# danini/multi-h

Measured on AMD Instinct MI355X. Metric: scored homography hypotheses/sec (50k pts x 100k models), higher is better.
Workload: dtype f64

## Files before the change

multi-h_amd/csrc/capi_label.hip:

```cpp
#include "capi_engine.hpp"

namespace {

int expand_contexts(const mh_engine* e)
{
    const int want = std::max(1, std::min(e->tune_expand_ctx, EXPAND_MAX_CTX));
    const double per_ctx = 4.0 * (2.0 * (double)e->g_nnz + 13.0 * (double)e->n + 2048.0);
    const int fit = 1 + (int)std::min(64.0, 8.0 * 1024.0 * 1024.0 * 1024.0 / std::max(per_ctx, 1.0));
    return std::max(1, std::min(want, fit));
}

int ensure_expand_work(mh_engine* e)
{
    const int n = e->n, n_ctx = expand_contexts(e);
    HIPCHK(e->ew_label.reserve(n));
    HIPCHK(e->ew_cur.reserve(n));
    HIPCHK(e->h_flags.ensure(EXPAND_HOST_WORDS));
    HIPCHK(e->h_acc.ensure(16));
    for (int k = 0; k < n_ctx; ++k) HIPCHK(e->ew_ctx[k].reserve(n, e->g_nnz, n_ctx > 1, e->stream));
    if (n_ctx > 1) {
        HIPCHK(e->ew_bctl.reserve(8 + EXPAND_MAX_CTX));
        HIPCHK(e->h_batch.ensure(8));
    }
    return MH_OK;
}

int do_data_cost(mh_engine* e)
{
    const int L = e->m + 1;
    HIPCHK(e->cost.reserve((size_t)e->n * L));
    {
        ScopedTimer t(e, MH_K_DATACOST);
        HIPCHK(launch_data_cost(e->pts(), e->H.p, e->m, e->lambda, e->thr_H * e->thr_H, e->cost.p, e->stream,
                                e->data_term == MH_DATA_TERM_RISING));
    }
    e->cost_L = L;
    return MH_OK;
}

int solve_grid_limit(mh_engine* e)
{
    if (e->solve_grid_max > 0) return MH_OK;
    int per_cu = 0;
    HIPCHK(solver_blocks_per_cu(&per_cu));
    if (per_cu < 1) return fail(MH_ERR_HIP, "the alpha-expansion solver kernel does not fit a compute unit");
    e->solve_grid_max = e->cu_count * 1;
    return MH_OK;
}

int do_expand(mh_engine* e, const int* init_dev, long long* energy, int* cycles)
{
    if (!e->have_graph) return fail(MH_ERR_NOT_SET, "neighbour graph is not set");
    if (e->cost_L != e->m + 1) return fail(MH_ERR_NOT_SET, "data cost is stale; call mh_data_cost first");
    int rc = ensure_expand_work(e);
    if (rc) return rc;
    Graph g{ e->d_rowptr.p, e->d_col.p, e->d_w.p, e->d_rev.p, e->n, e->g_nnz, e->d_order.p, e->d_wsum.p };
    rc = solve_grid_limit(e);
    if (rc) return rc;
    int solve_grid = std::max(1, std::min(e->tune_expand[3], e->solve_grid_max));
    ExpandWork w;
    w.label = e->ew_label.p; w.cur_cost = e->ew_cur.p;
    w.n_ctx = expand_contexts(e);
    for (int k = 0; k < w.n_ctx; ++k) w.ctx[k] = e->ew_ctx[k].view(g.n, g.nnz);
    w.h_flags = e->h_flags.h; w.h_flags_dev = e->h_flags.d;
    w.h_acc = e->h_acc.h; w.h_acc_dev = e->h_acc.d;
    if (w.n_ctx > 1) {
        w.bctl = e->ew_bctl.p;
        w.h_batch = e->h_batch.h; w.h_batch_dev = e->h_batch.d;
    }
    ExpandTuning& tu = w.tune;
    tu.relax_rounds = e->tune_expand[0]; tu.push_cycles = e->tune_expand[1]; tu.push_phases = e->tune_expand[2];
    tu.push_mult = e->tune_push_mult;
    tu.reduce_rounds = e->tune_reduce; tu.reduce_launches = e->tune_reduce_launches;
    tu.cascade_iters = e->tune_cascade_iters;
    tu.batch_min_labels = e->tune_batch_min_labels; tu.batch_spw = e->tune_batch_spw;
    const size_t recycle_words = (size_t)e->cost_L * ((size_t)g.nnz + (size_t)g.n);
    if (e->tune_recycle && recycle_words <= ((size_t)2 << 30)) {
        HIPCHK(e->ew_saved.reserve(recycle_words));
        HIPCHK(hipMemsetAsync(e->ew_saved.p, 0, sizeof(int) * recycle_words, e->stream));
        w.saved_flow = e->ew_saved.p;
        w.saved_sink = e->ew_saved.p + (size_t)e->cost_L * g.nnz;
    }
    if (e->trace_moves > 0) {
        HIPCHK(e->ew_trace.reserve(8 * (size_t)e->trace_moves + 4 * 2048));
        HIPCHK(hipMemsetAsync(e->ew_trace.p, 0, sizeof(int) * (8 * (size_t)e->trace_moves + 4 * 2048), e->stream));
        w.detail_move = e->detail_move;
        w.trace = e->ew_trace.p;
        w.trace_moves = e->trace_moves;
    }
    if (e->comp_moves > 0) {
        HIPCHK(e->ew_comp.reserve(2 * (size_t)g.n));
        HIPCHK(e->ew_comp_out.reserve(16 * (size_t)e->comp_moves));
        HIPCHK(hipMemsetAsync(e->ew_comp_out.p, 0, sizeof(int) * 16 * (size_t)e->comp_moves, e->stream));
        w.comp_out = e->ew_comp_out.p; w.comp_scratch = e->ew_comp.p; w.comp_moves = e->comp_moves;
    }
    const int potts = (int)std::round(100.0 * e->lambda);
    ExpandStats st{};
    {
        ScopedTimer t(e, MH_K_EXPAND);
        ExpandResult res;
        e->last_expand_retries = 0;
        for (int attempt = 0; attempt < 5; ++attempt) {
            tu.solve_grid = solve_grid;
            const bool last_attempt = attempt == 4 || solve_grid == 1;
            const double steady_ms = std::max(20.0, 50.0 * e->longest_barrier_wait_ms);
            tu.barrier_timeout_ticks = last_attempt ? 300000000ll : (long long)(steady_ms * 1e5);
            tu.barrier_first_timeout_ticks = last_attempt ? 300000000ll : (long long)(std::max(250.0, 10.0 * steady_ms) * 1e5);
            if (w.saved_flow) HIPCHK(hipMemsetAsync(e->ew_saved.p, 0, sizeof(int) * recycle_words, e->stream));
            HIPCHK(launch_init_labeling(e->cost.p, e->cost_L, e->n, init_dev, w.label, w.cur_cost, e->stream));
            w.hooks.inject_group = e->inject_solve_failure >> 4;
            w.hooks.inject_ctx = e->inject_solve_failure & 15;
            e->inject_solve_failure = 0;
            res = run_expansion(g, e->cost.p, e->cost_L, potts, w, 1000, &st, e->stream);
            if (res.status == ExpandStatus::ok && e->inject_barrier_timeouts > 0) {
                --e->inject_barrier_timeouts;
                res.status = ExpandStatus::barrier_timeout;
            }
            e->last_solve_grid = solve_grid;
            if (res.status != ExpandStatus::barrier_timeout || solve_grid == 1 || attempt == 4) break;
            if (attempt >= 1) solve_grid = std::max(1, solve_grid / 2);
            ++e->last_expand_retries;
            ++e->expand_retries_total;
        }
        switch (res.status) {
        case ExpandStatus::ok: break;
        case ExpandStatus::too_many_sites:
            return fail(MH_ERR_INVALID, "alpha-expansion: more sites than the solver's per-row state holds (about 1.3 million at 256 workgroups)");
        case ExpandStatus::overflow:
            return fail(MH_ERR_OVERFLOW, "int32 energy term overflow in alpha-expansion");
        case ExpandStatus::barrier_timeout:
            return fail(MH_ERR_HIP, "alpha-expansion: the solver's grid barrier timed out even with the launch cut down to a few workgroups "
                                    "(its workgroups were not all resident; is the GPU shared with other persistent launches?)");
        case ExpandStatus::no_convergence:
            return fail(MH_ERR_HIP, "alpha-expansion: push-relabel did not converge within its iteration bound");
        case ExpandStatus::hip_error: { const hipError_t he = res.hip; HIPCHK(he); }
        }
    }
    e->last_expand = st;
    if (st.max_barrier_wait_ms > e->longest_barrier_wait_ms) e->longest_barrier_wait_ms = std::min(st.max_barrier_wait_ms, 50.0);
    if (st.energy > 0x7fffffffll || st.energy < -0x7fffffffll)
        return fail(MH_ERR_OVERFLOW, "total energy exceeds the reference's int32 EnergyType");
    if (energy) *energy = st.energy;
    if (cycles) *cycles = st.cycles;
    return MH_OK;
}

__global__ void k_shift_labels(int n, const int* in, int delta, int* out)
{
    const int i = blockIdx.x * 256 + threadIdx.x;
    if (i < n) out[i] = in[i] + delta;
}

}

extern "C" {

static int compat_trial_stats(mh_engine* e, const double* pts_xyxy, const int* cluster_begin, int clusters, const int* tri,
                              const double* H, const unsigned char* ok, const double* F, int trials, double* stats_out, double* H_out,
                              unsigned char* ok_out)
{
    if (!e) return fail(MH_ERR_INVALID, "null engine");
    if (clusters < 0 || trials < 0) return fail(MH_ERR_INVALID, "negative cluster or trial count");
    if (clusters == 0 || trials == 0) return MH_OK;
    if (!pts_xyxy || !cluster_begin || !tri || !stats_out || (!F && (!H || !ok))) return fail(MH_ERR_INVALID, "null argument");
    if (cluster_begin[0] != 0) return fail(MH_ERR_INVALID, "cluster_begin[0] must be 0");
    for (int c = 0; c < clusters; ++c)
        if (cluster_begin[c + 1] - cluster_begin[c] < 19)
            return fail(MH_ERR_INVALID, "a cluster of fewer than 19 points: the caller handles those itself (the three stale entries of the reference's buffer reach the median ranks)");
    const size_t total = (size_t)cluster_begin[clusters], ct = (size_t)clusters * (size_t)trials;
    if (ct > (size_t)0x7fffffff) return fail(MH_ERR_INVALID, "too many trials");
    for (size_t i = 0; i < ct; ++i) {
        const int nc = cluster_begin[i / trials + 1] - cluster_begin[i / trials];
        for (int j = 0; j < 3; ++j)
            if (tri[3 * i + j] < 0 || tri[3 * i + j] >= nc) return fail(MH_ERR_INVALID, "a trial draws a point outside its cluster");
    }
    HIPCHK(hipSetDevice(e->device));
    HIPCHK(e->cp_pts.reserve(4 * total)); HIPCHK(e->cp_begin.reserve(clusters + 1)); HIPCHK(e->cp_tri.reserve(3 * ct));
    HIPCHK(e->cp_H.reserve(9 * ct)); HIPCHK(e->cp_ok.reserve(ct)); HIPCHK(e->cp_out.reserve(8 * ct));
    HIPCHK(hipMemcpyAsync(e->cp_pts.p, pts_xyxy, sizeof(double) * 4 * total, hipMemcpyHostToDevice, e->stream));
    HIPCHK(hipMemcpyAsync(e->cp_begin.p, cluster_begin, sizeof(int) * (clusters + 1), hipMemcpyHostToDevice, e->stream));
    HIPCHK(hipMemcpyAsync(e->cp_tri.p, tri, sizeof(int) * 3 * ct, hipMemcpyHostToDevice, e->stream));
    if (F) {
        HIPCHK(launch_compat_fit(e->cp_pts.p, e->cp_begin.p, clusters, e->cp_tri.p, F, trials, e->cp_H.p, e->cp_ok.p, e->stream));
    } else {
        HIPCHK(hipMemcpyAsync(e->cp_H.p, H, sizeof(double) * 9 * ct, hipMemcpyHostToDevice, e->stream));
        HIPCHK(hipMemcpyAsync(e->cp_ok.p, ok, ct, hipMemcpyHostToDevice, e->stream));
    }
    HIPCHK(launch_compat_select(e->cp_pts.p, e->cp_begin.p, clusters, e->cp_tri.p, e->cp_H.p, e->cp_ok.p, trials, e->cp_out.p, e->stream));
    HIPCHK(hipMemcpyAsync(stats_out, e->cp_out.p, sizeof(double) * 8 * ct, hipMemcpyDeviceToHost, e->stream));
    if (H_out) HIPCHK(hipMemcpyAsync(H_out, e->cp_H.p, sizeof(double) * 9 * ct, hipMemcpyDeviceToHost, e->stream));
    if (ok_out) HIPCHK(hipMemcpyAsync(ok_out, e->cp_ok.p, ct, hipMemcpyDeviceToHost, e->stream));
    HIPCHK(hipStreamSynchronize(e->stream));
    return MH_OK;
}

int mh_compat_trial_stats(mh_engine* e, const double* pts_xyxy, const int* cluster_begin, int clusters, const int* tri,
                          const double* H, const unsigned char* ok, int trials, double* stats_out)
{
    return guarded([&]() -> int {
    if (!H || !ok) return fail(MH_ERR_INVALID, "null argument");
    return compat_trial_stats(e, pts_xyxy, cluster_begin, clusters, tri, H, ok, nullptr, trials, stats_out, nullptr, nullptr);
    });
}

int mh_compat_trial_stats_fit(mh_engine* e, const double* pts_xyxy, const int* cluster_begin, int clusters, const int* tri,
                              const double F[9], int trials, double* stats_out, double* H_out, unsigned char* ok_out)
{
    return guarded([&]() -> int {
    if (!F) return fail(MH_ERR_INVALID, "null argument");
    return compat_trial_stats(e, pts_xyxy, cluster_begin, clusters, tri, nullptr, nullptr, F, trials, stats_out, H_out, ok_out);
    });
}

int mh_data_cost(mh_engine* e, int* cost)
{
    return guarded([&]() -> int {
    int rc = require_models(e);
    if (rc) return rc;
    rc = do_data_cost(e);
    if (rc) return rc;
    if (cost) {
        HIPCHK(hipMemcpyAsync(cost, e->cost.p, sizeof(int) * (size_t)e->n * e->cost_L, hipMemcpyDeviceToHost, e->stream));
        HIPCHK(hipStreamSynchronize(e->stream));
    }
    return MH_OK;
    });
}

int mh_expand(mh_engine* e, const int* init_labels, int* labels_out, int* energy, int* cycles)
{
    return guarded([&]() -> int {
    int rc = require_models(e);
    if (rc) return rc;
    const int* init_dev = nullptr;
    if (init_labels) {
        for (int i = 0; i < e->n; ++i)
            if (init_labels[i] < 0 || init_labels[i] > e->m)
                return fail(MH_ERR_INVALID, "initial label out of range 0..Nh");
        HIPCHK(e->labels_in.reserve(e->n));
        HIPCHK(hipMemcpyAsync(e->labels_in.p, init_labels, sizeof(int) * e->n, hipMemcpyHostToDevice, e->stream));
        init_dev = e->labels_in.p;
    }
    long long en = 0;
    rc = do_expand(e, init_dev, &en, cycles);
    if (rc) return rc;
    if (energy) *energy = (int)en;
    if (labels_out) {
        HIPCHK(hipMemcpyAsync(labels_out, e->ew_label.p, sizeof(int) * e->n, hipMemcpyDeviceToHost, e->stream));
        HIPCHK(hipStreamSynchronize(e->stream));
    }
    return MH_OK;
    });
}

int mh_get_expand_stats(mh_engine* e, long long stats[24])
{
    return guarded([&]() -> int {
    if (!e || !stats) return fail(MH_ERR_INVALID, "null argument");
    const ExpandStats& x = e->last_expand;
    stats[0] = x.cycles;
    stats[1] = x.moves;
    stats[2] = x.accepted;
    stats[3] = x.push_phases;
    stats[4] = x.relax_intervals;
    stats[5] = x.host_syncs;
    stats[6] = x.reduce_launches;
    stats[7] = x.flow_moves;
    stats[8] = x.launches;
    stats[9] = x.moves_run;
    stats[10] = x.moves_solved;
    stats[11] = x.core_sites;
    stats[12] = x.core_max;
    stats[13] = x.barriers;
    stats[14] = x.outer_iterations;
    stats[15] = (long long)(x.solve_ms * 1000.0);
    stats[16] = (long long)(x.barrier_ms * 1000.0);
    stats[17] = (long long)(x.relax_ms * 1000.0);
    stats[18] = (long long)(x.push_ms * 1000.0);
    stats[19] = (long long)(x.tail_ms * 1000.0);
    stats[20] = e->last_expand_retries;
    stats[21] = e->last_solve_grid;
    stats[22] = e->expand_retries_total;
    stats[23] = (long long)(e->last_expand.max_barrier_wait_ms * 1e3);
    return MH_OK;
    });
}

int mh_get_expand_batch_stats(mh_engine* e, long long stats[8])
{
    return guarded([&]() -> int {
    if (!e || !stats) return fail(MH_ERR_INVALID, "null argument");
    const ExpandStats& x = e->last_expand;
    stats[0] = x.batches;
    stats[1] = x.batch_committed;
    stats[2] = x.batch_invalid;
    stats[3] = x.host_skipped;
    stats[4] = x.solo_moves;
    stats[5] = x.injected_discarded;
    stats[6] = expand_contexts(e);
    stats[7] = e->tune_batch_min_labels;
    return MH_OK;
    });
}

int mh_get_expand_trace(mh_engine* e, int* trace, int moves)
{
    return guarded([&]() -> int {
    int rc = enter(e);
    if (rc) return rc;
    if (!trace || moves <= 0) return fail(MH_ERR_INVALID, "null trace or moves <= 0");
    if (e->trace_moves <= 0 || !e->ew_trace.p) return fail(MH_ERR_NOT_SET, "tracing is off (mh_set_tuning key 8) or no expansion has run");
    const int m = std::min(moves, (int)std::min<size_t>((size_t)e->trace_moves + 1024, e->ew_trace.cap / 8));
    HIPCHK(hipMemcpyAsync(trace, e->ew_trace.p, sizeof(int) * 8 * (size_t)m, hipMemcpyDeviceToHost, e->stream));
    HIPCHK(hipStreamSynchronize(e->stream));
    return MH_OK;
    });
}

int mh_get_core_components(mh_engine* e, int* out, int moves)
{
    return guarded([&]() -> int {
    int rc = enter(e);
    if (rc) return rc;
    if (!out || moves <= 0) return fail(MH_ERR_INVALID, "null output or moves <= 0");
    if (e->comp_moves <= 0 || !e->ew_comp_out.p) return fail(MH_ERR_NOT_SET, "the component diagnostic is off (mh_set_tuning key 21) or no expansion has run");
    const int m = std::min(moves, (int)(e->ew_comp_out.cap / 16));
    HIPCHK(hipMemcpyAsync(out, e->ew_comp_out.p, sizeof(int) * 16 * (size_t)m, hipMemcpyDeviceToHost, e->stream));
    HIPCHK(hipStreamSynchronize(e->stream));
    return MH_OK;
    });
}

}

namespace mhe {

int launch_estimator(mh_engine* e, const int* labels_dev, int Nh, double* H_dev, int* counts_dev)
{
    ScopedTimer t(e, MH_K_REESTIMATE);
    if (e->estimator == MH_ESTIMATOR_3PT) {
        HIPCHK(e->r3_scratch.reserve(reestimate_3pt_scratch_ints(e->n, Nh)));
        HIPCHK(launch_reestimate_3pt(e->pts(), labels_dev, Nh, e->epi, H_dev, counts_dev, e->r3_scratch.p, e->stream,
                                     e->tune_3pt_form));
        return MH_OK;
    }
    Affines a{ e->a11.p, e->a12.p, e->a21.p, e->a22.p };
    HIPCHK(launch_reestimate(e->pts(), a, labels_dev, Nh, e->epi, H_dev, counts_dev, e->stream));
    return MH_OK;
}

}

extern "C" {

int mh_set_estimator(mh_engine* e, int estimator)
{
    return guarded([&]() -> int {
    int rc = enter(e);
    if (rc) return rc;
    if (estimator != MH_ESTIMATOR_HAF && estimator != MH_ESTIMATOR_3PT) return fail(MH_ERR_INVALID, "unknown estimator");
    e->estimator = estimator;
    return MH_OK;
    });
}

int mh_set_data_term(mh_engine* e, int term)
{
    return guarded([&]() -> int {
    if (!e) return fail(MH_ERR_INVALID, "null engine");
    if (term != MH_DATA_TERM_REFERENCE && term != MH_DATA_TERM_RISING) return fail(MH_ERR_INVALID, "unknown data term");
    e->data_term = term;
    e->cost_L = 0;
    return MH_OK;
    });
}

int mh_reestimate(mh_engine* e, const int* labels, double* H_out)
{
    return guarded([&]() -> int {
    int rc = require_models(e);
    if (rc) return rc;
    if (!labels) return fail(MH_ERR_INVALID, "labels is null");
    if (e->estimator == MH_ESTIMATOR_HAF && !e->have_aff) return fail(MH_ERR_NOT_SET, "affinities are not set");
    if (!e->have_epi) return fail(MH_ERR_NOT_SET, "fundamental matrix / epipole are not set");
    HIPCHK(e->labels_pts.reserve(e->n));
    HIPCHK(e->label_counts.reserve(e->m));
    HIPCHK(hipMemcpyAsync(e->labels_pts.p, labels, sizeof(int) * e->n, hipMemcpyHostToDevice, e->stream));
    rc = launch_estimator(e, e->labels_pts.p, e->m, e->H.p, e->label_counts.p);
    if (rc) return rc;
    e->cost_L = 0;
    if (H_out) {
        HIPCHK(hipMemcpyAsync(H_out, e->H.p, sizeof(double) * 9 * e->m, hipMemcpyDeviceToHost, e->stream));
        HIPCHK(hipStreamSynchronize(e->stream));
    }
    return MH_OK;
    });
}

int mh_labeling_step(mh_engine* e, int warm, int* labeling, double* energy, int* cycles)
{
    return guarded([&]() -> int {
    int rc = require_models(e);
    if (rc) return rc;
    if (!labeling) return fail(MH_ERR_INVALID, "labeling is null");
    if (e->estimator == MH_ESTIMATOR_HAF && (!e->have_aff || !e->have_epi))
        return fail(MH_ERR_NOT_SET, "affinities / epipolar geometry are not set");
    if (!e->have_epi) return fail(MH_ERR_NOT_SET, "epipolar geometry is not set");
    rc = do_data_cost(e);
    if (rc) return rc;
    const int* init_dev = nullptr;
    const dim3 grid((e->n + 255) / 256), blk(256);
    if (warm) {
        for (int i = 0; i < e->n; ++i)
            if (labeling[i] < -1 || labeling[i] >= e->m)
                return fail(MH_ERR_INVALID, "warm-start label out of range -1..Nh-1");
        HIPCHK(e->labels_in.reserve(e->n));
        HIPCHK(hipMemcpyAsync(e->labels_in.p, labeling, sizeof(int) * e->n, hipMemcpyHostToDevice, e->stream));
        hipLaunchKernelGGL(k_shift_labels, grid, blk, 0, e->stream, e->n, e->labels_in.p, 1, e->labels_in.p);
        init_dev = e->labels_in.p;
    }
    long long en = 0;
    rc = do_expand(e, init_dev, &en, cycles);
    if (rc) return rc;
    HIPCHK(e->labels_pts.reserve(e->n));
    HIPCHK(e->label_counts.reserve(e->m));
    hipLaunchKernelGGL(k_shift_labels, grid, blk, 0, e->stream, e->n, e->ew_label.p, -1, e->labels_pts.p);
    rc = launch_estimator(e, e->labels_pts.p, e->m, e->H.p, e->label_counts.p);
    if (rc) return rc;
    e->cost_L = 0;
    HIPCHK(hipMemcpyAsync(labeling, e->labels_pts.p, sizeof(int) * e->n, hipMemcpyDeviceToHost, e->stream));
    HIPCHK(hipStreamSynchronize(e->stream));
    if (energy) *energy = (double)en;
    return MH_OK;
    });
}

}
```

multi-h_amd/csrc/expand.hip:

```cpp

#include "expand_ctl.hpp"
#include "expand_plan.hpp"

#include <algorithm>
#include <atomic>
#include <chrono>

namespace mh {

__global__ void k_ctl_init(MoveBatch b)
{
    int* flags = b.c[blockIdx.x].flags;
    long long* acc = b.c[blockIdx.x].acc;
    for (int t = threadIdx.x; t < C_COUNT; t += blockDim.x) flags[t] = (t == C_TLAST || t == C_PEND) ? -1 : 0;
    for (int t = threadIdx.x; t < A_TOTAL; t += blockDim.x) acc[t] = 0;
}

__global__ void __launch_bounds__(256)
k_init_labeling(const int* __restrict__ cost, int L, int n, const int* __restrict__ init,
                int* __restrict__ label, int* __restrict__ cur_cost)
{
    const int i = blockIdx.x * 256 + threadIdx.x;
    if (i >= n) return;
    const int l = init ? init[i] : 0;
    label[i] = l;
    cur_cost[i] = cost[(size_t)i * L + l];
}

__global__ void __launch_bounds__(256)
k_argmin_labels(const int* __restrict__ cost, int L, int n, int* __restrict__ label,
                long long* __restrict__ acc)
{
    const int i = blockIdx.x * 256 + threadIdx.x;
    long long mine = 0;
    if (i < n) {
        int best = 0, bc = cost[(size_t)i * L];
        for (int l = 1; l < L; ++l) {
            const int c = cost[(size_t)i * L + l];
            if (c < bc) { bc = c; best = l; }
        }
        label[i] = best;
        mine = bc;
    }
    __shared__ long long s[256];
    s[threadIdx.x] = mine;
    __syncthreads();
    for (int st = 128; st >= 1; st >>= 1) {
        if ((int)threadIdx.x < st) s[threadIdx.x] += s[threadIdx.x + st];
        __syncthreads();
    }
    if (threadIdx.x == 0)
        atomicAdd((unsigned long long*)&acc[A_ENERGY_S + (blockIdx.x % STRIPES) * STRIPE_LL], (unsigned long long)s[0]);
}

constexpr int LPN = 16;
constexpr int SITES_PER_BLOCK = 256 / LPN;


template <typename F>
__device__ __forceinline__ void for_flagged(unsigned long long mask, F body)
{
    const int grp = (int)(threadIdx.x & 63) / LPN;
    while (mask) {
        int b[4];
#pragma unroll
        for (int q = 0; q < 4; ++q) {
            b[q] = mask ? (int)__builtin_ctzll(mask) : -1;
            if (mask) mask &= mask - 1;
        }
        const int m = grp == 0 ? b[0] : grp == 1 ? b[1] : grp == 2 ? b[2] : b[3];
        body(m);
    }
}
constexpr int SPW = 16;
constexpr int SPW_MAX = 64;
constexpr int SITES_PER_WBLOCK_MAX = 4 * SPW_MAX;

__global__ void __launch_bounds__(256)
k_move_setup(Graph g, const int* __restrict__ cost, int L, int potts, int reduce_on,
             int* label, int* __restrict__ cur_cost, MoveBatch b, int spw)
{
    const MoveCtx& c = b.c[blockIdx.y];
    const int alpha = c.alpha, t = c.t;
    const unsigned char* __restrict__ took = c.took;
    int* __restrict__ cap = c.cap;
    int* __restrict__ excess = c.excess;
    int* __restrict__ sink_cap = c.sink_cap;
    int* __restrict__ decided = c.decided;
    int* __restrict__ flags = c.flags;
    long long* __restrict__ acc = c.acc;
    const int lane = threadIdx.x & 63;
    const int sub = threadIdx.x % LPN;
    const int s0 = (blockIdx.x * 4 + (int)(threadIdx.x >> 6)) * spw;
    const int i = s0 + lane;
    const bool in = lane < spw && i < g.n;
    const int pa = flags[C_PEND];
    int li = 0, cc = 0;
    if (in) {
        li = label[i];
        cc = cur_cost[i];
        if (pa >= 0 && took[i]) {
            li = pa;
            cc = cost[(size_t)i * L + pa];
            label[i] = pa; cur_cost[i] = cc;
        }
    }
    if (__shfl(move_is_skipped(flags, t, L) ? 1 : 0, 0)) return;
    long long K = 0;
    bool walk = false;
    if (in) {
        if (li == alpha) decided[i] = 3;
        else {
            K = cost[(size_t)i * L + alpha];
            if (reduce_on && K - cc > 2ll * potts * g.wsum[i]) decided[i] = 2;
            else walk = true;
        }
    }
    for_flagged(__ballot(walk), [&](int m) {
        const int mm = m < 0 ? 0 : m;
        const int li_m = __shfl(li, mm), cc_m = __shfl(cc, mm);
        const long long K_m = __shfl(K, mm);
        if (m < 0) return;
        const int im = s0 + m;
        const int k0 = g.rowptr[im], k1 = g.rowptr[im + 1];
        long long S = 0, out = 0, inn = 0;
        for (int k = k0 + sub; k < k1; k += LPN) {
            const int j = g.col[k];
            const long long wk64 = (long long)g.w[k] * potts;
            if (wk64 > 0x7fffffffll) atomicExch(&flags[C_ERROR], ERR_OVERFLOW);
            const int wk = wk64 > 0x7fffffffll ? 0x7fffffff : (int)wk64;
            int lj = label[j];
            if (pa >= 0 && took[j]) lj = pa;
            if (lj == alpha) { S += wk; cap[k] = 0; cap[g.rev[k]] = 0; }
            else if (j < im) { if (li_m != lj) S += wk; cap[k] = wk; out += wk; if (li_m == lj) inn += wk; }
            else { const int c = (li_m == lj) ? wk : 0; cap[k] = c; out += c; inn += wk; }
        }
        S = row_sum64<LPN>(S) + cc_m;
        out = row_sum64<LPN>(out);
        inn = row_sum64<LPN>(inn);
        if (sub != 0) return;
        const long long tr = S - K_m;
        if (tr > 0x7fffffffll || -tr > 0x7fffffffll) atomicExch(&flags[C_ERROR], ERR_OVERFLOW);
        const int ex = tr > 0 ? (int)tr : 0;
        excess[im] = ex;
        sink_cap[im] = tr < 0 ? (int)(-tr) : 0;
        int verdict = 0;
        if (reduce_on) {
            if (tr > out) verdict = 1;
            else if (-tr > inn) verdict = 2;
        }
        decided[im] = verdict;
        if (ex > 0) atomicAdd((unsigned long long*)&acc[A_EXCESS_S + (blockIdx.x % STRIPES) * STRIPE_LL], (unsigned long long)ex);
    });
}

template <bool COMPACT>
__global__ void __launch_bounds__(256)
k_reduce(Graph g, int L, MoveBatch b, int ROUNDS, int housekeep, int spw)
{
    const MoveCtx& c = b.c[blockIdx.y];
    const int t = c.t;
    int* cap = c.cap;
    int* excess = c.excess;
    int* sink_cap = c.sink_cap;
    int* decided = c.decided;
    int* __restrict__ flags = c.flags;
    long long* __restrict__ acc = c.acc;
    int* __restrict__ core = c.core;
    const int lane = threadIdx.x & 63;
    const int sub = threadIdx.x % LPN;
    const int slot = (blockIdx.x * 4 + (int)(threadIdx.x >> 6)) * spw + lane;
    const int u = (lane < spw && slot < g.n) ? (COMPACT ? g.order[slot] : slot) : -1;
    __shared__ int s_skip;
    __shared__ int s_cnt, s_base;
    __shared__ int s_list[SITES_PER_WBLOCK_MAX];
    if (threadIdx.x == 0) { s_skip = move_is_skipped(flags, t, L) ? 1 : 0; s_cnt = 0; }
    __syncthreads();
    const bool skipped = s_skip != 0;
    if (housekeep && blockIdx.x == 0 && threadIdx.x == 0) {
        flags[C_PEND] = -1;
        flags[C_TICKET] = 0;
        flags[C_TOOK_N] = 0;
        for (int s = 0; s < SUBTICKETS; ++s) flags[C_SUBTICKET + s * C_LINE] = 0;
        long long ex = 0;
        for (int s = 0; s < STRIPES; ++s) { ex += acc[A_EXCESS_S + s * STRIPE_LL]; acc[A_EXCESS_S + s * STRIPE_LL] = 0; acc[A_DELTA_S + s * STRIPE_LL] = 0; }
        if (!skipped && ex > 0x7fffffffll) flags[C_ERROR] = ERR_OVERFLOW;
    }
    if (skipped) return;
    const bool open = u >= 0 && LD(&decided[u]) == 0;
    for_flagged(__ballot(open), [&](int m) {
        const int um = __shfl(u, m < 0 ? 0 : m);
        if (m < 0) return;
        const int k0 = g.rowptr[um], k1 = g.rowptr[um + 1];
        long long net = (long long)excess[um] - sink_cap[um];
        bool dirty = false;
        int verdict = 0;
        for (int r = 0; r < ROUNDS; ++r) {
            long long add = 0, out = 0, in = 0;
            for (int k = k0 + sub; k < k1; k += LPN) {
                const int kr = g.rev[k];
                const int co = cap[k], ci = cap[kr];
                if ((co | ci) == 0) continue;
                const int dv = LD(&decided[g.col[k]]);
                if (dv == 1) { add += ci; cap[k] = 0; cap[kr] = 0; }
                else if (dv == 2) { add -= co; cap[k] = 0; cap[kr] = 0; }
                else { out += co; in += ci; }
            }
            add = row_sum64<LPN>(add); out = row_sum64<LPN>(out); in = row_sum64<LPN>(in);
            if (add != 0) { net += add; dirty = true; }
            if (net > out) verdict = 1;
            else if (-net > in) verdict = 2;
            if (verdict) break;
        }
        if (sub == 0) {
            if (dirty) {
                if (net > 0x7fffffffll || -net > 0x7fffffffll) atomicExch(&flags[C_ERROR], ERR_OVERFLOW);
                excess[um] = net > 0 ? (int)net : 0;
                sink_cap[um] = net < 0 ? (int)(-net) : 0;
            }
            if (verdict) ST(&decided[um], verdict);
            else if (COMPACT) s_list[atomicAdd(&s_cnt, 1)] = um;
        }
    });
    if (COMPACT) {
        __syncthreads();
        const int shard = blockIdx.x % EXPAND_CORE_SHARDS;
        if (threadIdx.x == 0 && s_cnt > 0) s_base = atomicAdd(&flags[C_CORE + shard], s_cnt);
        __syncthreads();
        if ((int)threadIdx.x < s_cnt) core[(size_t)shard * g.n + s_base + threadIdx.x] = s_list[threadIdx.x];
    }
}

__global__ void __launch_bounds__(1024)
k_core_components(Graph g, int L, int t, const int* __restrict__ decided, const int* __restrict__ flags, int* __restrict__ comp,
                  int* __restrict__ csize, int* __restrict__ out)
{
    __shared__ int s_changed, s_acc[16];
    if (threadIdx.x < 16) { s_acc[threadIdx.x] = 0; out[threadIdx.x] = 0; }
    if (move_is_skipped(flags, t, L)) return;
    for (int i = threadIdx.x; i < g.n; i += 1024) { comp[i] = decided[i] == 0 ? i : -1; csize[i] = 0; }
    __syncthreads();
    int rounds = 0;
    for (;;) {
        if (threadIdx.x == 0) s_changed = 0;
        __syncthreads();
        for (int i = threadIdx.x; i < g.n; i += 1024) {
            int c = comp[i];
            if (c < 0) continue;
            int m = c;
            for (int k = g.rowptr[i]; k < g.rowptr[i + 1]; ++k) { const int cj = comp[g.col[k]]; if (cj >= 0 && cj < m) m = cj; }
            if (m < c) { atomicMin(&comp[i], m); atomicMin(&comp[c], m); s_changed = 1; }
        }
        __syncthreads();
        for (int i = threadIdx.x; i < g.n; i += 1024) {
            int c = comp[i];
            if (c < 0) continue;
            while (comp[c] < c) c = comp[c];
            comp[i] = c;
        }
        __syncthreads();
        ++rounds;
        if (!s_changed || rounds > 4096) break;
        __syncthreads();
    }
    for (int i = threadIdx.x; i < g.n; i += 1024) if (comp[i] >= 0) { atomicAdd(&csize[comp[i]], 1); atomicAdd(&s_acc[0], 1); }
    __syncthreads();
    for (int i = threadIdx.x; i < g.n; i += 1024) {
        const int sz = csize[i];
        if (sz <= 0) continue;
        atomicAdd(&s_acc[1], 1);
        const int old = atomicMax(&s_acc[2], sz);
        atomicMax(&s_acc[3], old < sz ? old : sz);
        if (sz <= 64) { atomicAdd(&s_acc[4], sz); atomicAdd(&s_acc[9], 1); }
        if (sz <= 256) { atomicAdd(&s_acc[5], sz); atomicAdd(&s_acc[10], 1); }
        if (sz <= 1024) { atomicAdd(&s_acc[6], sz); atomicAdd(&s_acc[11], 1); }
        if (sz <= 2048) { atomicAdd(&s_acc[7], sz); atomicAdd(&s_acc[12], 1); }
        if (sz <= 8192) { atomicAdd(&s_acc[8], sz); atomicAdd(&s_acc[13], 1); }
    }
    __syncthreads();
    if (threadIdx.x < 16) out[threadIdx.x] = threadIdx.x == 14 ? rounds : s_acc[threadIdx.x];
}

__global__ void __launch_bounds__(256)
k_delta(Graph g, const int* __restrict__ cost, int L, int potts,
        const int* __restrict__ label, const int* __restrict__ cur_cost, MoveBatch b, int spw)
{
    const MoveCtx& c = b.c[blockIdx.y];
    const int alpha = c.alpha, t = c.t;
    const int* __restrict__ decided = c.decided;
    unsigned char* __restrict__ took = c.took;
    int* __restrict__ flags = c.flags;
    long long* acc = c.acc;
    __shared__ long long s[256];
    __shared__ int s_last;
    if (threadIdx.x == 0) s_last = move_is_skipped(flags, t, L) ? 1 : 0;
    __syncthreads();
    if (s_last) return;
    const int lane = threadIdx.x & 63;
    const int sub = threadIdx.x % LPN;
    const int s0 = (blockIdx.x * 4 + (int)(threadIdx.x >> 6)) * spw;
    const int i = s0 + lane;
    long long mine = 0;
    int oi = 0;
    bool ti = false;
    if (lane < spw && i < g.n) {
        oi = label[i];
        ti = decided[i] == 1;
        took[i] = ti ? 1 : 0;
        if (ti) mine += (long long)cost[(size_t)i * L + alpha] - cur_cost[i];
    }
    if (c.took_list) {
        const unsigned long long tb = __ballot(ti);
        if (tb) {
            int base = 0;
            if (lane == 0) base = atomicAdd(&flags[C_TOOK_N], (int)__popcll(tb));
            base = __shfl(base, 0);
            if (ti) c.took_list[base + (int)__popcll(tb & ((1ull << lane) - 1ull))] = i;
        }
    }
    for_flagged(__ballot(ti), [&](int m) {
        const int oi_m = __shfl(oi, m < 0 ? 0 : m);
        if (m < 0) return;
        const int im = s0 + m;
        for (int k = g.rowptr[im] + sub; k < g.rowptr[im + 1]; k += LPN) {
            const int j = g.col[k];
            const bool tj = decided[j] == 1;
            if (tj && j > im) continue;
            const int oj = label[j];
            const int nj = tj ? alpha : oj;
            const int dn = (alpha != nj) - (oi_m != oj);
            mine += (long long)dn * g.w[k] * potts;
        }
    });
    s[threadIdx.x] = mine;
    __syncthreads();
    for (int st = 128; st >= 1; st >>= 1) {
        if ((int)threadIdx.x < st) s[threadIdx.x] += s[threadIdx.x + st];
        __syncthreads();
    }
    if (threadIdx.x == 0) {
        if (s[0] != 0) atomicAdd((unsigned long long*)&acc[A_DELTA_S + (blockIdx.x % STRIPES) * STRIPE_LL], (unsigned long long)s[0]);
        asm volatile("s_waitcnt vmcnt(0)" ::: "memory");
        const int st = (int)(blockIdx.x % SUBTICKETS);
        const int members = ((int)gridDim.x - st + SUBTICKETS - 1) / SUBTICKETS;
        int last = 0;
        if (atomicAdd(&flags[C_SUBTICKET + st * C_LINE], 1) == members - 1) {
            const int used = (int)gridDim.x < SUBTICKETS ? (int)gridDim.x : SUBTICKETS;
            last = atomicAdd(&flags[C_TICKET], 1) == used - 1;
        }
        s_last = last;
    }
    __syncthreads();
    if (s_last && threadIdx.x < 64) {
        long long d = (int)threadIdx.x < STRIPES ? LD(&acc[A_DELTA_S + threadIdx.x * STRIPE_LL]) : 0ll;
#pragma unroll
        for (int m = 32; m >= 1; m >>= 1) d += __shfl_xor(d, m, 64);
        if (threadIdx.x == 0 && d < 0) {
            flags[C_TLAST] = t;
            flags[C_PEND] = alpha;
            flags[C_ACCEPTED] += 1;
        }
        if (threadIdx.x == 0) {
            flags[C_MOVES_RUN] += 1;
            for (int s = 0; s < EXPAND_CORE_SHARDS; ++s) flags[C_CORE + s] = 0;
            for (int s = C_XCD; s < C_TOP + C_LINE; ++s) flags[s] = 0;
            flags[C_ARRIVE] = 0;
        }
    }
}

__global__ void __launch_bounds__(256)
k_apply_pending(int n, const int* __restrict__ cost, int L, int* __restrict__ label,
                int* __restrict__ cur_cost, const unsigned char* __restrict__ took,
                const int* __restrict__ flags, int )
{
    const int pa = flags[C_PEND];
    if (pa < 0) return;
    const int i = blockIdx.x * 256 + threadIdx.x;
    if (i < n && took[i]) {
        label[i] = pa;
        cur_cost[i] = cost[(size_t)i * L + pa];
    }
}



__global__ void k_batch_prep(MoveBatch b, int* __restrict__ bctl)
{
    int* G = b.c[0].flags;
    const int k = threadIdx.x;
    if (k == 0) { bctl[B_TLAST0] = G[C_TLAST]; G[C_PEND] = -1; }
    if (k < EXPAND_MAX_CTX) bctl[B_BAD + k] = 0;
    if (k >= 1 && k < b.count) {
        int* f = b.c[k].flags;
        f[C_TLAST] = G[C_TLAST];
        f[C_PEND] = -1;
        f[C_ERROR] = G[C_ERROR];
    }
}

__device__ __forceinline__ bool batch_move_skipped(const MoveCtx& c, int tlast0, int L)
{
    return c.flags[C_ERROR] != 0 || (c.t >= L && tlast0 <= c.t - L);
}

__global__ void __launch_bounds__(256)
k_batch_check(Graph g, const int* __restrict__ cost, int L, int potts, const int* __restrict__ label, const int* __restrict__ cur_cost,
              MoveBatch b, int* __restrict__ bctl)
{
    const int j = blockIdx.y;
    if (j + 1 >= b.count) return;
    const MoveCtx& cj = b.c[j];
    const int tlast0 = bctl[B_TLAST0];
    if (batch_move_skipped(cj, tlast0, L) || cj.flags[C_PEND] < 0) return;
    const int nt = cj.flags[C_TOOK_N];
    const int sub = threadIdx.x % LPN;
    const int alpha_j = cj.alpha, later = b.count - 1 - j;
    unsigned bad = 0;
    for (int idx = blockIdx.x * SITES_PER_BLOCK + (int)threadIdx.x / LPN; idx < nt; idx += gridDim.x * SITES_PER_BLOCK) {
        const int p = cj.took_list[idx];
        const int k0 = g.rowptr[p], k1 = g.rowptr[p + 1];
        for (int a = k0 + sub - (sub == 0 ? 1 : 0); a < k1; a = (a < k0 ? k0 : a + LPN)) {
            const int s_ = a < k0 ? p : g.col[a];
            const long long W = (long long)potts * g.wsum[s_];
            const int lb = label[s_];
            const long long Dl = cur_cost[s_];
            const int* row = cost + (size_t)s_ * L + (alpha_j + 1);
            const long long Dj = a < k0 ? (long long)cost[(size_t)s_ * L + alpha_j] : 0;
            for (int q = 0; q < later; ++q) {
                const long long Db = row[q];
                bool ok = lb == alpha_j + 1 + q || Db - Dl > W;
                if (ok && a < k0) ok = Db - Dj > W;
                if (!ok) bad |= 1u << (j + 1 + q);
            }
        }
    }
#pragma unroll
    for (int m = 32; m >= 1; m >>= 1) bad |= (unsigned)__shfl_xor((int)bad, m, 64);
    if ((threadIdx.x & 63) == 0 && bad) atomicOr((unsigned*)&bctl[B_BAD + j], bad);
}

struct CtxFlags { int* p[EXPAND_MAX_CTX]; };
__global__ void __launch_bounds__(256)
k_batch_commit(const int* __restrict__ cost, int L, int* __restrict__ label, int* __restrict__ cur_cost, MoveBatch b,
               int* __restrict__ bctl, int* __restrict__ h_batch, CtxFlags all_flags, int n_ctx_all)
{
    __shared__ int s_first, s_err, s_last_t, s_n_acc;
    __shared__ unsigned s_acc;
    __shared__ int s_ek[EXPAND_MAX_CTX], s_pend[EXPAND_MAX_CTX], s_nt[EXPAND_MAX_CTX];
    __shared__ unsigned s_bad[EXPAND_MAX_CTX];
    __shared__ int s_g[5];
    if ((int)threadIdx.x < b.count) {
        const int* f = b.c[threadIdx.x].flags;
        s_ek[threadIdx.x] = f[C_ERROR];
        s_pend[threadIdx.x] = f[C_PEND];
        s_nt[threadIdx.x] = f[C_TOOK_N];
        s_bad[threadIdx.x] = (unsigned)bctl[B_BAD + threadIdx.x];
    } else if (threadIdx.x >= 64 && threadIdx.x < 69) {
        const int q = threadIdx.x - 64;
        const int* G = b.c[0].flags;
        s_g[q] = q == 0 ? bctl[B_TLAST0] : q == 1 ? G[C_ERROR] : q == 2 ? G[C_TLAST] : q == 3 ? G[C_ACCEPTED] : bctl[B_SEQ];
    }
    __syncthreads();
    if (threadIdx.x == 0) {
        const int tlast0 = s_g[0];
        unsigned accepted = 0;
        int first_invalid = b.count, err = 0, last_t = -1, n_acc = 0;
        for (int k = 0; k < b.count; ++k) {
            const MoveCtx& c = b.c[k];
            const int ek = s_ek[k];
            const bool skipped = ek != 0 || (c.t >= L && tlast0 <= c.t - L);
            bool valid = true;
            if (accepted) {
                if (skipped) valid = false;
                else
                    for (int j = 0; j < k; ++j)
                        if ((accepted >> j & 1u) && (s_bad[j] >> k & 1u)) valid = false;
            }
            if (!valid) { first_invalid = k; break; }
            if (ek) err = ek;
            if (!skipped && s_pend[k] >= 0) { accepted |= 1u << k; last_t = c.t; ++n_acc; }
        }
        s_first = first_invalid; s_err = err; s_acc = accepted; s_last_t = last_t; s_n_acc = n_acc;
    }
    __syncthreads();
    const unsigned accepted = s_acc;
    for (int k = 0; k < b.count; ++k) {
        if (!(accepted >> k & 1u)) continue;
        const MoveCtx& c = b.c[k];
        const int nt = s_nt[k], a = c.alpha;
        for (int i = blockIdx.x * 256 + threadIdx.x; i < nt; i += gridDim.x * 256) {
            const int p = c.took_list[i];
            label[p] = a;
            cur_cost[p] = cost[(size_t)p * L + a];
        }
    }
    __shared__ int s_is_last;
    __syncthreads();
    if (threadIdx.x == 0) {
        __threadfence();
        s_is_last = atomicAdd(&bctl[B_TICKET], 1) == (int)gridDim.x - 1;
    }
    __syncthreads();
    if (s_is_last && threadIdx.x == 0) {
        bctl[B_TICKET] = 0;
        int* G = b.c[0].flags;
        const int g_err = s_g[1] ? s_g[1] : s_err;
        const int g_tlast = s_last_t > s_g[2] ? s_last_t : s_g[2];
        const int seq = s_g[4] + 1;
        if (g_err != s_g[1]) G[C_ERROR] = g_err;
        if (g_tlast != s_g[2]) G[C_TLAST] = g_tlast;
        G[C_ACCEPTED] = s_g[3] + s_n_acc - (int)(accepted & 1u);
        bctl[B_SEQ] = seq;
        h_batch[HB_FIRST_INVALID] = s_first;
        h_batch[HB_TLAST] = g_tlast;
        h_batch[HB_ERROR] = g_err;
        h_batch[HB_ACCEPTED_HERE] = s_n_acc;
        h_batch[HB_DIRTY] = 0;
        __threadfence_system();
        __hip_atomic_store(&h_batch[HB_SEQ], seq, __ATOMIC_RELEASE, __HIP_MEMORY_SCOPE_SYSTEM);
        bctl[B_TLAST0] = g_tlast;
        G[C_PEND] = -1;
        for (int k = 0; k < EXPAND_MAX_CTX; ++k) bctl[B_BAD + k] = 0;
        for (int k = 1; k < n_ctx_all; ++k) {
            int* f = all_flags.p[k];
            f[C_TLAST] = g_tlast;
            f[C_PEND] = -1;
            f[C_ERROR] = g_err;
        }
    }
}

__global__ void k_stats_merge(MoveBatch b)
{
    const int t = threadIdx.x;
    int* G = b.c[0].flags;
    long long* A = b.c[0].acc;
    const int fw[5] = { C_FLOW_MOVES, C_MOVES_SOLVED, C_MOVES_RUN, C_CORE_MAX, C_XCD_USED };
    if (t < 5) {
        const int w = fw[t];
        int v = G[w];
        for (int k = 1; k < b.count; ++k) {
            int* f = b.c[k].flags;
            if (t < 3) v += f[w]; else if (f[w] > v) v = f[w];
            f[w] = 0;
        }
        G[w] = v;
    } else if (t >= 8 && t - 8 + A_CORE_SUM < A_COUNT) {
        const int w = t - 8 + A_CORE_SUM;
        long long v = A[w];
        for (int k = 1; k < b.count; ++k) {
            long long* a = b.c[k].acc;
            if (w == A_MAX_WAIT) { if (a[w] > v) v = a[w]; } else v += a[w];
            a[w] = 0;
        }
        A[w] = v;
    }
}

__global__ void __launch_bounds__(256)
k_energy(Graph g, int potts, const int* __restrict__ label, const int* __restrict__ cur_cost,
         int* __restrict__ flags, long long* __restrict__ acc)
{
    if (blockIdx.x == 0 && threadIdx.x == 0) flags[C_PEND] = -1;
    const int i = blockIdx.x * SITES_PER_BLOCK + threadIdx.x / LPN;
    const int sub = threadIdx.x % LPN;
    long long mine = 0;
    if (i < g.n) {
        if (sub == 0) mine = cur_cost[i];
        const int li = label[i];
        for (int k = g.rowptr[i] + sub; k < g.rowptr[i + 1]; k += LPN) {
            const int j = g.col[k];
            if (j < i && label[j] != li) mine += (long long)g.w[k] * potts;
        }
    }
    __shared__ long long s[256];
    s[threadIdx.x] = mine;
    __syncthreads();
    for (int st = 128; st >= 1; st >>= 1) {
        if ((int)threadIdx.x < st) s[threadIdx.x] += s[threadIdx.x + st];
        __syncthreads();
    }
    if (threadIdx.x == 0)
        atomicAdd((unsigned long long*)&acc[A_ENERGY_S + (blockIdx.x % STRIPES) * STRIPE_LL], (unsigned long long)s[0]);
}

hipError_t launch_init_labeling(const int* cost, int L, int n, const int* init, int* label,
                                int* cur_cost, hipStream_t s)
{
    hipLaunchKernelGGL(k_init_labeling, dim3((n + 255) / 256), dim3(256), 0, s, cost, L, n, init,
                       label, cur_cost);
    return hipGetLastError();
}

hipError_t launch_argmin_labels(const int* cost, int L, int n, int* label, long long* acc,
                                hipStream_t s)
{
    hipLaunchKernelGGL(k_argmin_labels, dim3((n + 255) / 256), dim3(256), 0, s, cost, L, n, label,
                       acc);
    return hipGetLastError();
}

__global__ void k_publish(const int* __restrict__ flags, long long* __restrict__ acc,
                          int* __restrict__ h_flags, long long* __restrict__ h_acc)
{
    const int t = threadIdx.x;
    if (t < EXPAND_HOST_WORDS) h_flags[t] = flags[t];
    long long en = t < STRIPES ? acc[A_ENERGY_S + t * STRIPE_LL] : 0ll;
    if (t < STRIPES) acc[A_ENERGY_S + t * STRIPE_LL] = 0;
#pragma unroll
    for (int m = 32; m >= 1; m >>= 1) en += __shfl_xor(en, m, 64);
    if (t < A_COUNT) h_acc[t] = t == A_ENERGY ? en : acc[t];
}

namespace {

ExpandResult hip_failed(hipError_t e) { return ExpandResult{ ExpandStatus::hip_error, e }; }
#define RET_IF(x) do { hipError_t e_ = (x); if (e_ != hipSuccess) return hip_failed(e_); } while (0)

struct Launcher {
    hipStream_t s;
    ExpandStats& stats;
    template <class... P, class... A>
    void operator()(void (*k)(P...), dim3 grid, dim3 blk, A&&... a) { ++stats.launches; uncounted(k, grid, blk, a...); }
    template <class... P, class... A>
    void uncounted(void (*k)(P...), dim3 grid, dim3 blk, A&&... a) { hipLaunchKernelGGL(k, grid, blk, 0, s, a...); }
    void solve(const SolveLaunch& sl, const Graph& g, int L, const MoveBatch& b, const SolveParams& sp)
    {
        ++stats.launches;
        launch_solve(sl, g, L, b, sp, s);
    }
};

hipError_t fetch(const ExpandWork& w, Launcher& launch)
{
    ++launch.stats.host_syncs;
    launch(k_publish, dim3(1), dim3(64), w.ctx[0].flags, w.ctx[0].acc, w.h_flags_dev, w.h_acc_dev);
    hipError_t e = hipGetLastError();
    return e != hipSuccess ? e : hipStreamSynchronize(launch.s);
}

hipError_t await_commit(const int* h_batch, int batch_seq, hipStream_t s)
{
    const volatile int* seq_word = h_batch + HB_SEQ;
    const auto t_poll = std::chrono::steady_clock::now();
    bool seen = false;
    for (int spin = 0;; ++spin) {
        if (*seq_word == batch_seq) { seen = true; break; }
        if ((spin & 255) == 255 && std::chrono::steady_clock::now() - t_poll > std::chrono::milliseconds(2)) break;
    }
    if (seen) std::atomic_thread_fence(std::memory_order_acquire);
    else if (hipError_t e = hipStreamSynchronize(s); e != hipSuccess) return e;
    return h_batch[HB_SEQ] == batch_seq ? hipSuccess : hipErrorUnknown;
}

ExpandStatus status_of(int err_word)
{
    return err_word == ERR_OVERFLOW ? ExpandStatus::overflow : err_word == ERR_BARRIER_TIMEOUT ? ExpandStatus::barrier_timeout
                                                                                               : ExpandStatus::no_convergence;
}

}

ExpandResult run_expansion(const Graph& g, const int* cost, int L, int potts, ExpandWork& w,
                           int max_cycles, ExpandStats* st, hipStream_t s)
{
    const ExpandTuning& tu = w.tune;
    const dim3 grid1((g.n + 255) / 256), blk(256);
    const dim3 grid((g.n + SITES_PER_BLOCK - 1) / SITES_PER_BLOCK);
    auto spw_for = [&](int count) {
        if (tu.batch_spw == 16 || tu.batch_spw == 32 || tu.batch_spw == 64) return tu.batch_spw;
        const long long site_moves = (long long)count * g.n;
        return site_moves > (1ll << 19) ? 64 : site_moves > (1ll << 18) ? 32 : 16;
    };
    ExpandStats stats = {};
    Launcher launch{ s, stats };
    auto ended = [&](ExpandStatus status) { if (st) *st = stats; return ExpandResult{ status, hipSuccess }; };
    const int n_ctx = std::max(1, std::min(w.n_ctx, EXPAND_MAX_CTX));
    MoveBatch all{};
    all.count = n_ctx;
    CtxFlags all_flags{};
    for (int k = 0; k < n_ctx; ++k) {
        const ExpandWork::Ctx& x = w.ctx[k];
        MoveCtx& c = all.c[k];
        c.cap = x.cap; c.sent = x.sent; c.excess = x.excess; c.sink_cap = x.sink_cap; c.height = x.height; c.decided = x.decided;
        c.took = x.took; c.core = x.core; c.flags = x.flags; c.acc = x.acc; c.took_list = x.took_list;
        all_flags.p[k] = x.flags;
    }
    const ExpandWork::Ctx& ctx0 = w.ctx[0];
    launch(k_ctl_init, dim3(n_ctx), dim3(64), all);
    RET_IF(hipGetLastError());
    auto finish_cycle = [&]() -> hipError_t {
        if (n_ctx > 1) launch(k_stats_merge, dim3(1), dim3(64), all);
        return fetch(w, launch);
    };

    if (g.nnz == 0) {
        RET_IF(launch_argmin_labels(cost, L, g.n, w.label, ctx0.acc, s));
        RET_IF(fetch(w, launch));
        stats.energy = w.h_acc[A_ENERGY];
        return ended(ExpandStatus::ok);
    }

    long long energy = 0, old_energy = 0;
    launch(k_energy, grid, blk, g, potts, w.label, w.cur_cost, ctx0.flags, ctx0.acc);
    RET_IF(fetch(w, launch));
    energy = w.h_acc[A_ENERGY];
    if (energy > 0x7fffffffll)
        return ended(ExpandStatus::overflow);

    const SolveParams sp{ tu.reduce_rounds, tu.relax_rounds, tu.push_cycles, tu.push_phases, tu.push_mult > 0 ? tu.push_mult : 1, 1 << 20, tu.cascade_iters,
                          tu.barrier_timeout_ticks > 0 ? (unsigned long long)tu.barrier_timeout_ticks : 300000000ull,
                          tu.barrier_first_timeout_ticks > 0 ? (unsigned long long)tu.barrier_first_timeout_ticks : 300000000ull };
    SolveLaunch sl;
    RET_IF(prepare_solve(g.n, tu.solve_grid > 0 ? tu.solve_grid : 128, &sl));
    if (!sl.fits) return ExpandResult{ ExpandStatus::too_many_sites, hipSuccess };

    bool prepared = false;
    int group = 0;
    int injected_ctx = -1;
    auto enqueue_moves = [&](int alpha0, int t0, int count, int cycle) -> hipError_t {
        MoveBatch b = all;
        b.count = count;
        for (int k = 0; k < count; ++k) {
            MoveCtx& c = b.c[k];
            c.alpha = alpha0 + k;
            c.t = t0 + k;
            c.trace = (w.trace && c.t < w.trace_moves) ? w.trace : nullptr;
            c.detail = (w.trace && c.t == w.detail_move) ? w.trace + 8 * (size_t)w.trace_moves : nullptr;
            c.saved_flow = w.saved_flow ? w.saved_flow + (size_t)c.alpha * g.nnz : nullptr;
            c.saved_sink = w.saved_flow ? w.saved_sink + (size_t)c.alpha * g.n : nullptr;
            c.warm = (w.saved_flow && cycle > 1) ? 1 : 0;
            if (count == 1) c.took_list = nullptr;
        }
        const int spw = count > 1 ? spw_for(count) : SPW;
        const int spw_d = count > 1 ? SPW_MAX : SPW;
        const dim3 grid_w((unsigned)((g.n + 4 * spw - 1) / (4 * spw)), (unsigned)count);
        const dim3 grid_d((unsigned)((g.n + 4 * spw_d - 1) / (4 * spw_d)), (unsigned)count);
        if (count > 1 && !prepared) launch(k_batch_prep, dim3(1), dim3(64), b, w.bctl);
        prepared = count > 1;
        launch(k_move_setup, grid_w, blk, g, cost, L, potts, tu.reduce_rounds > 0 ? 1 : 0, w.label, w.cur_cost, b, spw);
        if (tu.reduce_launches > 1) launch(k_reduce<false>, grid_w, blk, g, L, b, tu.reduce_rounds, 1, spw);
        launch(k_reduce<true>, grid_w, blk, g, L, b, tu.reduce_rounds, tu.reduce_launches > 1 ? 0 : 1, spw);
        if (tu.reduce_rounds > 0) stats.reduce_launches += tu.reduce_launches > 1 ? 2 : 1;
        if (count == 1 && w.comp_out && t0 < w.comp_moves)
            launch.uncounted(k_core_components, dim3(1), dim3(1024), g, L, t0, ctx0.decided, ctx0.flags, w.comp_scratch,
                             w.comp_scratch + g.n, w.comp_out + 16 * (size_t)t0);
        launch.solve(sl, g, L, b, sp);
        injected_ctx = -1;
        if (++group == w.hooks.inject_group && w.hooks.inject_ctx < count) {
            if (hipError_t e = hipMemsetD32Async((hipDeviceptr_t)(b.c[w.hooks.inject_ctx].flags + C_ERROR), ERR_NO_CONVERGENCE, 1, s); e != hipSuccess) return e;
            injected_ctx = w.hooks.inject_ctx;
        }
        launch(k_delta, grid_d, blk, g, cost, L, potts, w.label, w.cur_cost, b, spw_d);
        if (count > 1) {
            launch(k_batch_check, dim3(32, (unsigned)count), blk, g, cost, L, potts, w.label, w.cur_cost, b, w.bctl);
            launch(k_batch_commit, dim3(32), blk, cost, L, w.label, w.cur_cost, b, w.bctl, w.h_batch_dev, all_flags, n_ctx);
        }
        return hipGetLastError();
    };

    const bool can_batch = n_ctx > 1 && w.bctl && w.h_batch && L >= 2 && !w.comp_out;
    if (can_batch) {
        RET_IF(hipMemsetAsync(w.bctl, 0, sizeof(int) * B_WORDS, s));
        w.h_batch[HB_SEQ] = 0;
    }
    ExpandPlan plan(L, can_batch ? n_ctx : 1, tu.batch_min_labels);
    int batch_seq = 0;
    for (;;) {
        old_energy = energy;
        while (!plan.cycle_done()) {
            const ExpandPlan::Step step = plan.next();
            if (step.kind == ExpandPlan::Kind::skip_rest) {
                stats.moves += step.count; stats.host_skipped += step.count;
                continue;
            }
            if (step.kind == ExpandPlan::Kind::solo) {
                RET_IF(enqueue_moves(step.alpha, step.t, 1, plan.cycle()));
                ++stats.moves; ++stats.solo_moves;
                continue;
            }
            if (step.apply_pending) launch(k_apply_pending, grid1, blk, g.n, cost, L, w.label, w.cur_cost, ctx0.took, ctx0.flags, 1);
            RET_IF(enqueue_moves(step.alpha, step.t, step.count, plan.cycle()));
            ++stats.batches;
            ++stats.host_syncs;
            RET_IF(await_commit(w.h_batch, ++batch_seq, s));
            if (w.h_batch[HB_ERROR]) break;
            const int j = w.h_batch[HB_FIRST_INVALID];
            if (injected_ctx >= j) ++stats.injected_discarded;
            stats.moves += j; stats.batch_committed += j;
            if (j < step.count) ++stats.batch_invalid;
            plan.committed(j, w.h_batch[HB_TLAST]);
        }
        launch(k_apply_pending, grid1, blk, g.n, cost, L, w.label, w.cur_cost, ctx0.took, ctx0.flags, 0);
        launch(k_energy, grid, blk, g, potts, w.label, w.cur_cost, ctx0.flags, ctx0.acc);
        RET_IF(finish_cycle());
        stats.cycles = plan.cycle();
        if (w.h_flags[C_ERROR]) return ended(status_of(w.h_flags[C_ERROR]));
        plan.cycle_ended(w.h_flags[C_TLAST]);
        energy = w.h_acc[A_ENERGY];
        if (energy == old_energy || plan.cycle() > max_cycles) break;
    }
    stats.energy = energy;
    stats.accepted = w.h_flags[C_ACCEPTED];
    stats.flow_moves = w.h_flags[C_FLOW_MOVES];
    stats.moves_solved = w.h_flags[C_MOVES_SOLVED];
    stats.moves_run = w.h_flags[C_MOVES_RUN];
    stats.core_sites = w.h_acc[A_CORE_SUM];
    stats.core_max = w.h_flags[C_CORE_MAX];
    stats.outer_iterations = w.h_acc[A_OUTER];
    stats.relax_intervals = w.h_acc[A_RELAX];
    stats.push_phases = w.h_acc[A_PUSH];
    stats.barriers = w.h_acc[A_BARRIERS];
    stats.solve_ms = (double)w.h_acc[A_TICKS] * 1e-5;
    stats.barrier_ms = (double)w.h_acc[A_T_BAR] * 1e-5;
    stats.relax_ms = (double)w.h_acc[A_T_RELAX] * 1e-5;
    stats.push_ms = (double)w.h_acc[A_T_PUSH] * 1e-5;
    stats.tail_ms = (double)w.h_acc[A_T_TAIL] * 1e-5;
    stats.tail_rounds = w.h_acc[A_TAIL_ROUNDS];
    stats.max_barrier_wait_ms = (double)w.h_acc[A_MAX_WAIT] * 1e-5;
    return ended(ExpandStatus::ok);
}

}
```

Baseline: 13.27 million.

## Fuse batch conflict check into delta kernel and drop recycle buffer memset

Moves the per-context batch interference test into k_delta, so each took site and its neighbours are tested against later contexts' labels while already being visited, and removes the separate k_batch_check launch that re-walked the took list. It also drops the zeroing memset of the saved-flow recycle buffer. In exchange, k_delta does extra per-edge work whenever later contexts exist, including for neighbours that are skipped. The check no longer applies the skipped-move and pending guards the old kernel had, and the recycle buffer may now hold stale data.

```diff
diff --git a/multi-h_amd/csrc/capi_label.hip b/multi-h_amd/csrc/capi_label.hip
--- a/multi-h_amd/csrc/capi_label.hip
+++ b/multi-h_amd/csrc/capi_label.hip
@@ -77,7 +77,6 @@
     const size_t recycle_words = (size_t)e->cost_L * ((size_t)g.nnz + (size_t)g.n);
     if (e->tune_recycle && recycle_words <= ((size_t)2 << 30)) {
         HIPCHK(e->ew_saved.reserve(recycle_words));
-        HIPCHK(hipMemsetAsync(e->ew_saved.p, 0, sizeof(int) * recycle_words, e->stream));
         w.saved_flow = e->ew_saved.p;
         w.saved_sink = e->ew_saved.p + (size_t)e->cost_L * g.nnz;
     }
diff --git a/multi-h_amd/csrc/expand.hip b/multi-h_amd/csrc/expand.hip
--- a/multi-h_amd/csrc/expand.hip
+++ b/multi-h_amd/csrc/expand.hip
@@ -281,12 +281,25 @@
     if (threadIdx.x < 16) out[threadIdx.x] = threadIdx.x == 14 ? rounds : s_acc[threadIdx.x];
 }
 
+__device__ __forceinline__ unsigned batch_test(const int* __restrict__ row, int later, int lq, long long Dl, long long W, bool self, long long Dj)
+{
+    unsigned bad = 0;
+    for (int q = 0; q < later; ++q) {
+        const long long Db = row[q];
+        bool ok = lq == q || Db - Dl > W;
+        if (ok && self) ok = Db - Dj > W;
+        if (!ok) bad |= 1u << q;
+    }
+    return bad;
+}
+
 __global__ void __launch_bounds__(256)
 k_delta(Graph g, const int* __restrict__ cost, int L, int potts,
-        const int* __restrict__ label, const int* __restrict__ cur_cost, MoveBatch b, int spw)
+        const int* __restrict__ label, const int* __restrict__ cur_cost, MoveBatch b, int* __restrict__ bctl, int spw)
 {
     const MoveCtx& c = b.c[blockIdx.y];
     const int alpha = c.alpha, t = c.t;
+    const int later = b.count - 1 - (int)blockIdx.y;
     const int* __restrict__ decided = c.decided;
     unsigned char* __restrict__ took = c.took;
     int* __restrict__ flags = c.flags;
@@ -303,11 +316,17 @@
     long long mine = 0;
     int oi = 0;
     bool ti = false;
+    unsigned bad = 0;
     if (lane < spw && i < g.n) {
         oi = label[i];
         ti = decided[i] == 1;
         took[i] = ti ? 1 : 0;
-        if (ti) mine += (long long)cost[(size_t)i * L + alpha] - cur_cost[i];
+        if (ti) {
+            const long long Dj = cost[(size_t)i * L + alpha], Dl = cur_cost[i];
+            mine += Dj - Dl;
+            if (later > 0)
+                bad = batch_test(cost + (size_t)i * L + (alpha + 1), later, oi - (alpha + 1), Dl, (long long)potts * g.wsum[i], true, Dj);
+        }
     }
     if (c.took_list) {
         const unsigned long long tb = __ballot(ti);
@@ -325,13 +344,20 @@
         for (int k = g.rowptr[im] + sub; k < g.rowptr[im + 1]; k += LPN) {
             const int j = g.col[k];
             const bool tj = decided[j] == 1;
+            const int oj = label[j];
+            if (later > 0)
+                bad |= batch_test(cost + (size_t)j * L + (alpha + 1), later, oj - (alpha + 1), cur_cost[j], (long long)potts * g.wsum[j], false, 0);
             if (tj && j > im) continue;
-            const int oj = label[j];
             const int nj = tj ? alpha : oj;
             const int dn = (alpha != nj) - (oi_m != oj);
             mine += (long long)dn * g.w[k] * potts;
         }
     });
+    if (later > 0) {
+#pragma unroll
+        for (int m = 32; m >= 1; m >>= 1) bad |= (unsigned)__shfl_xor((int)bad, m, 64);
+        if (lane == 0 && bad) atomicOr((unsigned*)&bctl[B_BAD + blockIdx.y], bad << (blockIdx.y + 1));
+    }
     s[threadIdx.x] = mine;
     __syncthreads();
     for (int st = 128; st >= 1; st >>= 1) {
@@ -397,47 +423,6 @@
         f[C_PEND] = -1;
         f[C_ERROR] = G[C_ERROR];
     }
-}
-
-__device__ __forceinline__ bool batch_move_skipped(const MoveCtx& c, int tlast0, int L)
-{
-    return c.flags[C_ERROR] != 0 || (c.t >= L && tlast0 <= c.t - L);
-}
-
-__global__ void __launch_bounds__(256)
-k_batch_check(Graph g, const int* __restrict__ cost, int L, int potts, const int* __restrict__ label, const int* __restrict__ cur_cost,
-              MoveBatch b, int* __restrict__ bctl)
-{
-    const int j = blockIdx.y;
-    if (j + 1 >= b.count) return;
-    const MoveCtx& cj = b.c[j];
-    const int tlast0 = bctl[B_TLAST0];
-    if (batch_move_skipped(cj, tlast0, L) || cj.flags[C_PEND] < 0) return;
-    const int nt = cj.flags[C_TOOK_N];
-    const int sub = threadIdx.x % LPN;
-    const int alpha_j = cj.alpha, later = b.count - 1 - j;
-    unsigned bad = 0;
-    for (int idx = blockIdx.x * SITES_PER_BLOCK + (int)threadIdx.x / LPN; idx < nt; idx += gridDim.x * SITES_PER_BLOCK) {
-        const int p = cj.took_list[idx];
-        const int k0 = g.rowptr[p], k1 = g.rowptr[p + 1];
-        for (int a = k0 + sub - (sub == 0 ? 1 : 0); a < k1; a = (a < k0 ? k0 : a + LPN)) {
-            const int s_ = a < k0 ? p : g.col[a];
-            const long long W = (long long)potts * g.wsum[s_];
-            const int lb = label[s_];
-            const long long Dl = cur_cost[s_];
-            const int* row = cost + (size_t)s_ * L + (alpha_j + 1);
-            const long long Dj = a < k0 ? (long long)cost[(size_t)s_ * L + alpha_j] : 0;
-            for (int q = 0; q < later; ++q) {
-                const long long Db = row[q];
-                bool ok = lb == alpha_j + 1 + q || Db - Dl > W;
-                if (ok && a < k0) ok = Db - Dj > W;
-                if (!ok) bad |= 1u << (j + 1 + q);
-            }
-        }
-    }
-#pragma unroll
-    for (int m = 32; m >= 1; m >>= 1) bad |= (unsigned)__shfl_xor((int)bad, m, 64);
-    if ((threadIdx.x & 63) == 0 && bad) atomicOr((unsigned*)&bctl[B_BAD + j], bad);
 }
 
 struct CtxFlags { int* p[EXPAND_MAX_CTX]; };
@@ -752,9 +737,8 @@
             if (hipError_t e = hipMemsetD32Async((hipDeviceptr_t)(b.c[w.hooks.inject_ctx].flags + C_ERROR), ERR_NO_CONVERGENCE, 1, s); e != hipSuccess) return e;
             injected_ctx = w.hooks.inject_ctx;
         }
-        launch(k_delta, grid_d, blk, g, cost, L, potts, w.label, w.cur_cost, b, spw_d);
+        launch(k_delta, grid_d, blk, g, cost, L, potts, w.label, w.cur_cost, b, w.bctl, spw_d);
         if (count > 1) {
-            launch(k_batch_check, dim3(32, (unsigned)count), blk, g, cost, L, potts, w.label, w.cur_cost, b, w.bctl);
             launch(k_batch_commit, dim3(32), blk, cost, L, w.label, w.cur_cost, b, w.bctl, w.h_batch_dev, all_flags, n_ctx);
         }
         return hipGetLastError();
```

Measured after the change: 13.33 million, median of 2. About the same (+0.5%).
